# LingmaFuture/PRCV2025REID

Hardware: AMD Instinct MI355X
Metric: multimodal instances/sec (PxK, 5-modality) at 1/2/4/8 GPU; eval queries/sec (higher is better)
Workload: dtype bf16

## Files before the change

### prcv2025reid_amd/csrc/common.h

```cpp
#pragma once
#include <hip/hip_runtime.h>
#include <stdint.h>
#include <stdio.h>
#include "../../include/reid_hip.h"

typedef __attribute__((ext_vector_type(8))) short bf16x8;
typedef __attribute__((ext_vector_type(4))) short bf16x4;
typedef __attribute__((ext_vector_type(4))) float f32x4;
typedef __attribute__((ext_vector_type(16))) float f32x16;
typedef unsigned short bf16_t;

__attribute__((visibility("hidden"))) void reid_set_error(const char* fmt, ...);

enum reid_knob_id { KNOB_GEMM_TILE, KNOB_ATTN_BWD, KNOB_LORA_IMPL, KNOB_LN_IMPL, KNOB_TOPK_TILE, KNOB_TOPK_SCAN, KNOB_COUNT };
__attribute__((visibility("hidden"))) int reid_knob(int id);
__attribute__((visibility("hidden"))) int reid_num_cus();

#define REID_CHECK_ARG(cond, ...)                     \
    do {                                              \
        if (!(cond)) {                                \
            reid_set_error(__VA_ARGS__);              \
            return REID_ERR_ARG;                      \
        }                                             \
    } while (0)

static inline hipError_t reid_max_dyn_lds(const void* fn, int bytes, unsigned* done_mask) {
    int dev = 0;
    hipError_t e = hipGetDevice(&dev);
    if (e != hipSuccess) return e;
    if (dev >= 0 && dev < 32 && ((__atomic_load_n(done_mask, __ATOMIC_ACQUIRE) >> dev) & 1u)) return hipSuccess;
    e = hipFuncSetAttribute(fn, hipFuncAttributeMaxDynamicSharedMemorySize, bytes);
    if (e == hipSuccess && dev >= 0 && dev < 32) __atomic_fetch_or(done_mask, 1u << dev, __ATOMIC_RELEASE);
    return e;
}
#define REID_MAX_LDS(kernel, bytes)                                                                              \
    do {                                                                                                         \
        static unsigned lds_done_ = 0;                                                                           \
        const hipError_t le_ = reid_max_dyn_lds((const void*)(kernel), (int)(bytes), &lds_done_);                \
        if (le_ != hipSuccess) {                                                                                 \
            reid_set_error("hipFuncSetAttribute(%s, dynamic LDS %d): %s", #kernel, (int)(bytes), hipGetErrorString(le_)); \
            return REID_ERR_LAUNCH;                                                                              \
        }                                                                                                        \
    } while (0)

#define REID_CHECK_HIP(call, what)                                                     \
    do {                                                                               \
        const hipError_t he_ = (call);                                                 \
        if (he_ != hipSuccess) {                                                       \
            reid_set_error("%s: %s", what, hipGetErrorString(he_));                    \
            return REID_ERR_LAUNCH;                                                    \
        }                                                                              \
    } while (0)

#define REID_CHECK_LAUNCH(name)                                                        \
    do {                                                                               \
        hipError_t e_ = hipGetLastError();                                             \
        if (e_ != hipSuccess) {                                                        \
            reid_set_error("%s: launch failed: %s", name, hipGetErrorString(e_));     \
            return REID_ERR_LAUNCH;                                                    \
        }                                                                              \
    } while (0)

typedef _Float16 __attribute__((ext_vector_type(8))) half8_t;
#ifdef REID_FLAVOR_F16
__device__ __forceinline__ float bf16_to_f32(bf16_t v) { return (float)__builtin_bit_cast(_Float16, v); }
__device__ __forceinline__ bf16_t f32_to_bf16(float f) { return __builtin_bit_cast(bf16_t, (_Float16)f); }
__device__ __forceinline__ f32x4 mfma16(bf16x8 a, bf16x8 b, f32x4 c) {
    return __builtin_amdgcn_mfma_f32_16x16x32_f16(__builtin_bit_cast(half8_t, a), __builtin_bit_cast(half8_t, b), c, 0, 0, 0);
}
__device__ __forceinline__ f32x16 mfma32(bf16x8 a, bf16x8 b, f32x16 c) {
    return __builtin_amdgcn_mfma_f32_32x32x16_f16(__builtin_bit_cast(half8_t, a), __builtin_bit_cast(half8_t, b), c, 0, 0, 0);
}
#define REID_T16_ENTER() __builtin_amdgcn_s_setreg(1 | (23 << 6) | (0 << 11), 1)
#define REID_FLAVOR_ID 1
#define REID_T16_EPS 0.0009765625f
#else
__device__ __forceinline__ float bf16_to_f32(bf16_t v) { return __uint_as_float(((uint32_t)v) << 16); }
__device__ __forceinline__ bf16_t f32_to_bf16(float f) {
    __bf16 b = (__bf16)f;
    return __builtin_bit_cast(bf16_t, b);
}
__device__ __forceinline__ f32x4 mfma16(bf16x8 a, bf16x8 b, f32x4 c) { return __builtin_amdgcn_mfma_f32_16x16x32_bf16(a, b, c, 0, 0, 0); }
__device__ __forceinline__ f32x16 mfma32(bf16x8 a, bf16x8 b, f32x16 c) { return __builtin_amdgcn_mfma_f32_32x32x16_bf16(a, b, c, 0, 0, 0); }
#define REID_T16_ENTER() do { } while (0)
#define REID_FLAVOR_ID 0
#define REID_T16_EPS 0.00390625f
#endif

typedef float pk_f32x2 __attribute__((ext_vector_type(2)));
#ifdef REID_FLAVOR_F16
typedef _Float16 pk_t16x2 __attribute__((ext_vector_type(2)));
#else
typedef __bf16 pk_t16x2 __attribute__((ext_vector_type(2)));
#endif
__device__ __forceinline__ uint32_t pack_bf16x2(float lo, float hi) {
    const pk_t16x2 r = __builtin_convertvector(pk_f32x2{lo, hi}, pk_t16x2);
    return __builtin_bit_cast(uint32_t, r);
}

typedef _Float16 pk_h16x2 __attribute__((ext_vector_type(2)));
__device__ __forceinline__ uint32_t pack_f16x2(float lo, float hi) {
    const pk_h16x2 r = __builtin_convertvector(pk_f32x2{lo, hi}, pk_h16x2);
    return __builtin_bit_cast(uint32_t, r);
}
__device__ __forceinline__ float f16_to_f32(unsigned short v) { return (float)__builtin_bit_cast(_Float16, v); }
#define REID_F16_SATURATE() __builtin_amdgcn_s_setreg(1 | (23 << 6) | (0 << 11), 1)
__device__ __forceinline__ bool f16_clamps(float v) { const float a = fabsf(v); return a >= 65520.f && a <= 3.402823466e38f; }

__device__ __forceinline__ float wave_sum(float v) {
#pragma unroll
    for (int o = 32; o > 0; o >>= 1) v += __shfl_xor(v, o, 64);
    return v;
}
__device__ __forceinline__ float wave_max(float v) {
#pragma unroll
    for (int o = 32; o > 0; o >>= 1) v = fmaxf(v, __shfl_xor(v, o, 64));
    return v;
}

__device__ __forceinline__ void gauss_cdf_pdf(float x, float& cdf, float& pdf_unnorm) {
    const float z = fabsf(x) * 0.70710678118654752f;
    const float t = __builtin_amdgcn_rcpf(fmaf(0.3275911f, z, 1.0f));
    const float e = __builtin_amdgcn_exp2f(x * x * -0.72134752044448170f);
    const float poly = t * fmaf(t, fmaf(t, fmaf(t, fmaf(t, 1.061405429f, -1.453152027f), 1.421413741f), -0.284496736f), 0.254829592f);
    const float q = 0.5f * poly * e;
    cdf = x >= 0.f ? 1.0f - q : q;
    pdf_unnorm = e;
}
__device__ __forceinline__ float gelu_erf_f(float x) {
    float c, e;
    gauss_cdf_pdf(x, c, e);
    return x * c;
}
__device__ __forceinline__ void gelu_both_f(float x, float& g, float& dg) {
    float c, e;
    gauss_cdf_pdf(x, c, e);
    g = x * c;
    dg = fmaf(x * 0.39894228040143268f, e, c);
}
typedef float f32x2_t __attribute__((ext_vector_type(2)));
__device__ __forceinline__ void gelu_both_x2(f32x2_t x, f32x2_t& g, f32x2_t& dg) {
    const f32x2_t xs = (x * x) * -0.72134752044448170f;
    f32x2_t e; e.x = __builtin_amdgcn_exp2f(xs.x); e.y = __builtin_amdgcn_exp2f(xs.y);
    f32x2_t z; z.x = __builtin_fabsf(x.x); z.y = __builtin_fabsf(x.y);
    const f32x2_t den = z * (0.3275911f * 0.70710678118654752f) + 1.0f;
    f32x2_t t; t.x = __builtin_amdgcn_rcpf(den.x); t.y = __builtin_amdgcn_rcpf(den.y);
    f32x2_t poly = t * (0.5f * 1.061405429f) + (0.5f * -1.453152027f);
    poly = poly * t + (0.5f * 1.421413741f);
    poly = poly * t + (0.5f * -0.284496736f);
    poly = poly * t + (0.5f * 0.254829592f);
    const f32x2_t q = (poly * t) * e;
    const f32x2_t h = 0.5f - q;
    f32x2_t sh; sh.x = __builtin_copysignf(h.x, x.x); sh.y = __builtin_copysignf(h.y, x.y);
    const f32x2_t cdf = sh + 0.5f;
    g = x * cdf;
    dg = (x * 0.39894228040143268f) * e + cdf;
}
__device__ __forceinline__ float dgelu_erf_f(float x) {
    float c, e;
    gauss_cdf_pdf(x, c, e);
    return fmaf(x * 0.39894228040143268f, e, c);
}
__device__ __forceinline__ float quick_gelu_f(float x) { return x / (1.0f + __expf(-1.702f * x)); }
__device__ __forceinline__ float dquick_gelu_f(float x) {
    const float s = 1.0f / (1.0f + __expf(-1.702f * x));
    return s + x * 1.702f * s * (1.0f - s);
}
// ... 1 lines not shown
```

### prcv2025reid_amd/csrc/gemm.hip

```cpp
#include "gemm_core.h"
#include <stdlib.h>
#include <type_traits>

namespace {

struct GemmParams {
    const bf16_t* A; const bf16_t* B; const bf16_t* A2; const bf16_t* B2;
    const float* bias; const void* R; const bf16_t* aux;
    void* C; void* C2;
    const int32_t* img_mod;
    const float* row_scale;
    int M, N, K, K2;
    int lda, ldb, lda2, ldb2, ldr, ldaux, ldc, ldc2;
    int k2_group_n;
    int act, c_dtype, c2_dtype, r_dtype;
    int r_period;
    int mask_r, mask_period, rows_per_img;
    int c_group, c_group_stride, c_row_off;
    float alpha;
    int tiles_m, tiles_n;
    int group_m;
    int perm_b;
    int epi;
    int n_groups;
// ... 301 lines not shown
    if (!p.perm_b || p.R || p.row_scale) return EPI_GENERIC;
    if (p.act == REID_ACT_NONE && !p.C2 && !p.aux) return p.c_dtype == REID_F16 ? EPI_PLAIN16H : EPI_PLAIN16;
    if (p.act == REID_ACT_GELU_ERF && p.C2 && p.c2_dtype != REID_F32 && !p.aux) return EPI_GELU2;
    if (p.act == REID_ACT_DGELU_ERF && p.aux && !p.C2) return EPI_DGELU;
    if (p.act == REID_ACT_GELU_ERF_DSAVE && p.C2 && p.c2_dtype != REID_F32 && !p.aux) return EPI_GELU2D;
    if (p.act == REID_ACT_MUL_AUX && p.aux && !p.C2) return EPI_MULAUX;
    return EPI_GENERIC;
}

__host__ __device__ inline bool epilogue_wide16(const GemmParams& p) {
    return p.c_dtype != REID_F32 && ((p.N | p.ldc) & 7) == 0 && (!p.C2 || (p.ldc2 & 7) == 0) && (!p.R || (p.ldr & 7) == 0) &&
           (!p.aux || (p.ldaux & 7) == 0);
}

template <int TM, int TN>
__device__ __forceinline__ void store_tile(const GemmParams& p, f32x4 (&acc)[TN][TM], int m_base, int n_base, int lane, int m_end) {
    if (p.c_dtype == REID_F32) store_tile_m<TM, TN, 0>(p, acc, m_base, n_base, lane, m_end);
    else if (p.perm_b) store_tile_m<TM, TN, 1>(p, acc, m_base, n_base, lane, m_end);
    else store_tile_m<TM, TN, 2>(p, acc, m_base, n_base, lane, m_end);
}

template <int BM, int BN, int WM, int WN, int EPI = EPI_GENERIC>
__global__ __launch_bounds__(WM* WN * 64, 2) void mer_gemm_kernel(const GemmParams p) {
    REID_T16_ENTER();
    using C = Cfg<BM, BN, WM, WN>;
    if constexpr (EPI == EPI_PLAIN16H) REID_F16_SATURATE();
    extern __shared__ __attribute__((aligned(16))) char smem[];
    const int tid = threadIdx.x;
    const int lane = tid & 63;
    const int wave = __builtin_amdgcn_readfirstlane(tid >> 6);
    const int wm = wave / WN, wn = wave % WN;

    const int lin = xcd_linear_block(blockIdx.x, gridDim.x);
    int tm, tn;
    tile_coords(lin, p.tiles_m, p.tiles_n, tm, tn, p.group_m);
    int m0, m_end;
    const bf16_t* Bw;
    tile_rows(p, tm, BM, m0, m_end, Bw);
    const int n0 = tn * BN;
    const int g = (p.k2_group_n > 0) ? (n0 / p.k2_group_n) : 0;
    const bf16_t* A2 = p.A2 ? p.A2 + (size_t)g * p.K2 : nullptr;

    f32x4 acc[C::TN][C::TM];
    if constexpr (EPI == EPI_GENERIC) init_acc<C::TM, C::TN>(p, acc, n0 + wn * (BN / WN), lane);
    else if constexpr (EPI == EPI_RES32) init_acc_m<C::TM, C::TN, 0>(p, acc, n0 + wn * (BN / WN), lane);
    else init_acc_m<C::TM, C::TN, 1>(p, acc, n0 + wn * (BN / WN), lane);
    mainloop<BM, BN, WM, WN>(p.A, p.lda, Bw, p.ldb, A2, p.lda2, p.B2, p.ldb2, m_end, p.N, p.K, p.K2, m0, n0, smem, acc,
                             p.perm_b != 0);

    constexpr int WTM = BM / WM, WTN = BN / WN;
    if constexpr (EPI == EPI_GENERIC) store_tile<C::TM, C::TN>(p, acc, m0 + wm * WTM, n0 + wn * WTN, lane, m_end);
    else store_tile_fast<C::TM, C::TN, EPI>(p, acc, m0 + wm * WTM, n0 + wn * WTN, lane, m_end);
}

template <int EPI, int BM = 256>
__global__ __launch_bounds__(512, 2) void mer_gemm_pp_kernel(const GemmParams p) {
    REID_T16_ENTER();
    if constexpr (EPI == EPI_PLAIN16H) REID_F16_SATURATE();
    using PC = PPCfg<BM, 256>;
    constexpr int TM = PC::TM, RW = PC::RW;
    extern __shared__ __attribute__((aligned(16))) char smem[];
    const int tid = threadIdx.x;
    const int lane = tid & 63;
    const int wave = __builtin_amdgcn_readfirstlane(tid >> 6);
    const int wm = wave >> 2, wn = wave & 3;
#ifdef REID_GEMM_TRACE
#define GEMM_TRACE(slot) do { if (p.trace && threadIdx.x == 0) p.trace[(size_t)blockIdx.x * 8 + (slot)] = __builtin_amdgcn_s_memrealtime(); } while (0)
    if (p.trace && threadIdx.x == 0) p.trace[(size_t)blockIdx.x * 8 + 6] = ((unsigned long long)__builtin_amdgcn_s_getreg(20 | (0 << 6) | (31 << 11)) << 32) | __builtin_amdgcn_s_getreg(4 | (0 << 6) | (31 << 11));
#else
#define GEMM_TRACE(slot) do { } while (0)
#endif
    GEMM_TRACE(0);
    const int lin = xcd_linear_block(blockIdx.x, gridDim.x);
    int tm, tn;
    tile_coords(lin, p.tiles_m, p.tiles_n, tm, tn, p.group_m);
    int m0, m_end;
    const bf16_t* Bw;
    tile_rows(p, tm, BM, m0, m_end, Bw);
    const int n0 = tn * 256;
    const int g = (p.k2_group_n > 0) ? (n0 / p.k2_group_n) : 0;
    const bf16_t* A2 = p.A2 ? p.A2 + (size_t)g * p.K2 : nullptr;
    f32x4 acc[4][TM];
    if constexpr (EPI == EPI_GENERIC) init_acc<TM, 4>(p, acc, n0 + wn * 64, lane);
    else if constexpr (EPI == EPI_RES32) init_acc_m<TM, 4, 0>(p, acc, n0 + wn * 64, lane);
    else init_acc_m<TM, 4, 1>(p, acc, n0 + wn * 64, lane);
    constexpr bool AUX_IN_LOOP = EPI == EPI_MULAUX && BM == 256;
    const bool aux_staged = AUX_IN_LOOP && p.K2 == 0 && (p.K >> 6) >= 2;
    mainloop_pp<BM, 256, AUX_IN_LOOP>(p.A, p.lda, Bw, p.ldb, A2, p.lda2, p.B2, p.ldb2, m_end, p.N, p.K, p.K2, m0, n0, smem, acc, p.perm_b != 0,
                                      aux_staged ? (const bf16_t*)p.aux : nullptr, p.ldaux);
    GEMM_TRACE(1);
    if constexpr (EPI == EPI_MULAUX) {
        if (aux_staged) {
            asm volatile("s_waitcnt vmcnt(0)" ::: "memory");
            __syncthreads();
            store_tile_fast<TM, 4, EPI>(p, acc, m0 + wm * RW, n0 + wn * 64, lane, m_end, smem, wm * RW, wn * 8);
            GEMM_TRACE(2);
#ifdef REID_GEMM_TRACE
            asm volatile("s_waitcnt vmcnt(0)" ::: "memory");
            GEMM_TRACE(3);
#endif
            return;
        }
        __syncthreads();
#pragma unroll
        for (int q = 0; q < BM / 16; ++q) {
            const int rp = q * 8 + wave;
            const int row = 2 * rp + (lane >> 5);
            const int c = lane & 31;
            const int gm = m0 + row < m_end ? m0 + row : m_end - 1;
            const char* src = (const char*)p.aux + ((size_t)gm * p.ldaux + n0) * 2 + ((c ^ (row & 15)) << 4);
            __builtin_amdgcn_global_load_lds((gptr_t)src, (lptr_t)(smem + rp * 1024), 16, 0, 0);
        }
        asm volatile("s_waitcnt vmcnt(0)" ::: "memory");
        __syncthreads();
        store_tile_fast<TM, 4, EPI>(p, acc, m0 + wm * RW, n0 + wn * 64, lane, m_end, smem, wm * RW, wn * 8);
        GEMM_TRACE(2);
#ifdef REID_GEMM_TRACE
        asm volatile("s_waitcnt vmcnt(0)" ::: "memory");
        GEMM_TRACE(3);
#endif
        return;
    }
    if constexpr (EPI == EPI_GENERIC) store_tile<TM, 4>(p, acc, m0 + wm * RW, n0 + wn * 64, lane, m_end);
    else store_tile_fast<TM, 4, EPI>(p, acc, m0 + wm * RW, n0 + wn * 64, lane, m_end);
    GEMM_TRACE(2);
#ifdef REID_GEMM_TRACE
    asm volatile("s_waitcnt vmcnt(0)" ::: "memory");
    GEMM_TRACE(3);
#endif
}
#ifdef REID_GEMM_TRACE
static unsigned long long* g_gemm_trace = nullptr;
extern "C" void reid_debug_gemm_trace(void* buf) { g_gemm_trace = (unsigned long long*)buf; }
#endif

template <int EPI, int BM = 256>
__global__ __launch_bounds__(512, 2) void mer_gemm_pps_kernel(const GemmParams p) {
    REID_T16_ENTER();
    if constexpr (EPI == EPI_PLAIN16H) REID_F16_SATURATE();
    using PC = PPCfg<BM, 256>;
    constexpr int TM = PC::TM, RW = PC::RW;
    extern __shared__ __attribute__((aligned(16))) char smem[];
    const int lane = threadIdx.x & 63;
    const int wave = __builtin_amdgcn_readfirstlane(threadIdx.x >> 6);
    const int wm = wave >> 2, wn = wave & 3;
    const int n_tiles = p.tiles_m * p.tiles_n;
    auto tile_of = [&](int v, int& m0, int& m_end, int& n0, const bf16_t*& Bw) {
        const int lin = xcd_linear_block(v, n_tiles);
        int tm, tn;
        tile_coords(lin, p.tiles_m, p.tiles_n, tm, tn, p.group_m);
        tile_rows(p, tm, BM, m0, m_end, Bw);
        n0 = tn * 256;
    };
    auto init = [&](f32x4 (&acc)[4][TM], int n0) {
        if constexpr (EPI == EPI_RES32) init_acc_m<TM, 4, 0>(p, acc, n0 + wn * 64, lane);
        else init_acc_m<TM, 4, 1>(p, acc, n0 + wn * 64, lane);
    };
    auto epi = [&](f32x4 (&acc)[4][TM], int m0, int m_end, int n0) {
        store_tile_fast<TM, 4, EPI>(p, acc, m0 + wm * RW, n0 + wn * 64, lane, m_end);
    };
#ifdef REID_GEMM_TRACE
    auto trace = [&](int v, int slot) {
        if (!p.trace) return;
        if (threadIdx.x == 0) {
            p.trace[(size_t)v * 8 + slot] = __builtin_amdgcn_s_memrealtime();
#ifndef REID_GEMM_TRACE_CLOCK
            if (slot == 0) p.trace[(size_t)v * 8 + 7] = ((unsigned long long)__builtin_amdgcn_s_getreg(20 | (0 << 6) | (31 << 11)) << 32) | __builtin_amdgcn_s_getreg(4 | (0 << 6) | (31 << 11));
#endif
        }
#ifdef REID_GEMM_TRACE_CLOCK
        if (threadIdx.x == 0 && slot == 1) p.trace[(size_t)v * 8 + 6] = __builtin_amdgcn_s_memtime();
        if (threadIdx.x == 0 && slot == 2) p.trace[(size_t)v * 8 + 7] = __builtin_amdgcn_s_memtime();
#else
        if (threadIdx.x == 256 && slot == 5) p.trace[(size_t)v * 8 + 6] = __builtin_amdgcn_s_memrealtime();
#endif
    };
#else
    auto trace = [&](int, int) {};
#endif
    stream_pp<BM, 256>(p.A, p.lda, p.ldb, p.N, p.K, n_tiles, smem, p.perm_b != 0, tile_of, init, epi, trace);
}

template <int EPI, int BM>
int launch_pps_e(GemmParams& p, hipStream_t s) {
    using C = PPCfg<BM, 256>;
    constexpr int LDS = C::LDS_BYTES;
    REID_MAX_LDS((mer_gemm_pps_kernel<EPI, BM>), LDS);
    const int tiles = p.tiles_m * p.tiles_n;
    int grid = reid_num_cus() & ~7;
    if (grid > tiles) grid = tiles;
#ifdef REID_GEMM_TRACE
    p.trace = g_gemm_trace;
#endif
    hipLaunchKernelGGL((mer_gemm_pps_kernel<EPI, BM>), dim3(grid), dim3(C::NT), LDS, s, p);
    REID_CHECK_LAUNCH("reid_mer_gemm");
    return REID_OK;
}


template <int EPI, int BM>
int launch_pp_e(GemmParams& p, hipStream_t s) {
    using C = PPCfg<BM, 256>;
    REID_MAX_LDS((mer_gemm_pp_kernel<EPI, BM>), C::LDS_BYTES);
    hipLaunchKernelGGL((mer_gemm_pp_kernel<EPI, BM>), dim3(p.tiles_m * p.tiles_n), dim3(C::NT), C::LDS_BYTES, s, p);
    REID_CHECK_LAUNCH("reid_mer_gemm");
    return REID_OK;
}
static int pick_pp_bm(const GemmParams& p, int tile_knob) {
    if (tile_knob == 12) return 256;
    if (tile_knob == 14) return 224;
    const long cus = reid_num_cus();
    const long tn = p.N / 256;
    GemmParams q = p;
    const long t256 = (long)row_tiles(q, 256, false) * tn, t224 = (long)row_tiles(q, 224, false) * tn;
    return (t224 + cus - 1) / cus <= (t256 + cus - 1) / cus ? 224 : 256;
}
int launch_pp(GemmParams& p, hipStream_t s, int tile_knob) {
    p.epi = pick_epilogue(p, 256);
    const int bm = p.epi == EPI_GENERIC ? 256 : pick_pp_bm(p, tile_knob);
    p.tiles_m = row_tiles(p, bm, true);
    p.tiles_n = (p.N + 255) / 256;
#ifdef REID_GEMM_TRACE
    p.trace = g_gemm_trace;
#endif
    if (p.K2 == 0 && p.K >= 192 && (reid_num_cus() & ~7) >= 8) {
        switch (p.epi) {
            case EPI_PLAIN16: return bm == 224 ? launch_pps_e<EPI_PLAIN16, 224>(p, s) : launch_pps_e<EPI_PLAIN16, 256>(p, s);
#ifndef REID_FLAVOR_F16
            case EPI_PLAIN16H: return bm == 224 ? launch_pps_e<EPI_PLAIN16H, 224>(p, s) : launch_pps_e<EPI_PLAIN16H, 256>(p, s);
#endif
            case EPI_RES32: return bm == 224 ? launch_pps_e<EPI_RES32, 224>(p, s) : launch_pps_e<EPI_RES32, 256>(p, s);
            default: break;
        }
    }
#define REID_PP_CASE(E) case E: return bm == 224 ? launch_pp_e<E, 224>(p, s) : launch_pp_e<E, 256>(p, s);
    switch (p.epi) {
        REID_PP_CASE(EPI_PLAIN16)
#ifndef REID_FLAVOR_F16
        REID_PP_CASE(EPI_PLAIN16H)
#endif
        REID_PP_CASE(EPI_RES32)
        REID_PP_CASE(EPI_GELU2)
        REID_PP_CASE(EPI_DGELU)
        REID_PP_CASE(EPI_GELU2D)
        REID_PP_CASE(EPI_MULAUX)
        default: return launch_pp_e<EPI_GENERIC, 256>(p, s);
    }
#undef REID_PP_CASE
}

template <int BM, int BN, int WM, int WN, int EPI>
int launch_e(GemmParams& p, hipStream_t s) {
    using C = Cfg<BM, BN, WM, WN>;
    REID_MAX_LDS((mer_gemm_kernel<BM, BN, WM, WN, EPI>), C::LDS_BYTES);
    hipLaunchKernelGGL((mer_gemm_kernel<BM, BN, WM, WN, EPI>), dim3(p.tiles_m * p.tiles_n), dim3(C::NT), C::LDS_BYTES, s, p);
    REID_CHECK_LAUNCH("reid_mer_gemm");
    return REID_OK;
}
int launch_main(GemmParams& p, hipStream_t s) {
    p.tiles_m = row_tiles(p, 128, true);
    p.tiles_n = (p.N + 127) / 128;
    p.epi = pick_epilogue(p, 128);
    switch (p.epi) {
        case EPI_PLAIN16: return launch_e<128, 128, 2, 2, EPI_PLAIN16>(p, s);
#ifndef REID_FLAVOR_F16
        case EPI_PLAIN16H: return launch_e<128, 128, 2, 2, EPI_PLAIN16H>(p, s);
#endif
        case EPI_RES32: return launch_e<128, 128, 2, 2, EPI_RES32>(p, s);
        case EPI_GELU2: return launch_e<128, 128, 2, 2, EPI_GELU2>(p, s);
        case EPI_DGELU: return launch_e<128, 128, 2, 2, EPI_DGELU>(p, s);
        case EPI_GELU2D: return launch_e<128, 128, 2, 2, EPI_GELU2D>(p, s);
        case EPI_MULAUX: return launch_e<128, 128, 2, 2, EPI_MULAUX>(p, s);
        default: return launch_e<128, 128, 2, 2, EPI_GENERIC>(p, s);
    }
}

template <int BM, int BN, int WM, int WN>
int launch(GemmParams& p, hipStream_t s) {
    using C = Cfg<BM, BN, WM, WN>;
    p.tiles_m = row_tiles(p, BM, true);
    p.tiles_n = (p.N + BN - 1) / BN;
    REID_MAX_LDS((mer_gemm_kernel<BM, BN, WM, WN>), C::LDS_BYTES);
    const int grid = p.tiles_m * p.tiles_n;
    hipLaunchKernelGGL((mer_gemm_kernel<BM, BN, WM, WN>), dim3(grid), dim3(C::NT), C::LDS_BYTES, s, p);
    REID_CHECK_LAUNCH("reid_mer_gemm");
    return REID_OK;
}

}

extern "C" int reid_mer_gemm(const reid_gemm_args* a, void* stream) {
    REID_CHECK_ARG(a != nullptr, "reid_mer_gemm: null args");
    REID_CHECK_ARG(a->A && a->B && a->C, "reid_mer_gemm: A, B, C must be non-null");
    REID_CHECK_ARG(a->M > 0 && a->N > 0 && a->K > 0, "reid_mer_gemm: empty problem M=%d N=%d K=%d", a->M, a->N, a->K);
    REID_CHECK_ARG(a->K % 64 == 0, "reid_mer_gemm: K=%d must be a multiple of 64", a->K);
    REID_CHECK_ARG(a->N % 4 == 0, "reid_mer_gemm: N=%d must be a multiple of 4", a->N);
    REID_CHECK_ARG(a->lda >= a->K && a->ldb >= a->K && a->lda % 8 == 0 && a->ldb % 8 == 0,
                   "reid_mer_gemm: lda/ldb must be >= K and multiples of 8 (16-byte rows)");
    REID_CHECK_ARG(a->ldc >= a->N && a->ldc % 4 == 0, "reid_mer_gemm: ldc=%d", a->ldc);
    REID_CHECK_ARG((int64_t)a->M * a->lda * 2 < (1ll << 32) && (int64_t)a->N * a->ldb * 2 < (1ll << 32),
                   "reid_mer_gemm: operands beyond 4 GiB need 64-bit lane offsets (M*lda=%lld)", (long long)a->M * a->lda);
    if (a->A2) {
        REID_CHECK_ARG(a->B2 && a->K2 > 0 && a->K2 % 32 == 0, "reid_mer_gemm: K2=%d must be a positive multiple of 32",
                       a->K2);
        REID_CHECK_ARG(a->lda2 % 8 == 0 && a->ldb2 % 8 == 0 && a->ldb2 >= a->K2, "reid_mer_gemm: lda2/ldb2");
        const int groups = a->k2_group_n > 0 ? (a->N + a->k2_group_n - 1) / a->k2_group_n : 1;
        REID_CHECK_ARG(a->lda2 >= groups * a->K2, "reid_mer_gemm: lda2=%d < groups*K2=%d", a->lda2, groups * a->K2);
        REID_CHECK_ARG(a->k2_group_n == 0 || a->k2_group_n % 128 == 0, "reid_mer_gemm: k2_group_n must be a multiple of 128");
    }
    REID_CHECK_ARG(a->act >= 0 && a->act <= REID_ACT_GELU_ERF_DSAVE, "reid_mer_gemm: act=%d", a->act);
    REID_CHECK_ARG(a->act < REID_ACT_DGELU_ERF || a->act > REID_ACT_MUL_AUX || (a->aux && a->ldaux >= a->N), "reid_mer_gemm: D* / MUL_AUX activation needs aux");
    REID_CHECK_ARG(a->act != REID_ACT_GELU_ERF_DSAVE || a->C2, "reid_mer_gemm: GELU_ERF_DSAVE needs C2");
    REID_CHECK_ARG(!a->R || a->ldr >= a->N, "reid_mer_gemm: ldr");
    REID_CHECK_ARG(!a->C2 || a->ldc2 >= a->N, "reid_mer_gemm: ldc2");
    REID_CHECK_ARG(a->mask_r == 0 || (a->img_mod && a->rows_per_img > 0 && a->mask_period > 0),
                   "reid_mer_gemm: modality mask needs img_mod, rows_per_img, mask_period");
    REID_CHECK_ARG(a->c_group == 0 || a->c_group_stride >= a->c_group, "reid_mer_gemm: c_group_stride");
    REID_CHECK_ARG(!a->row_scale || a->rows_per_img > 0, "reid_mer_gemm: row_scale needs rows_per_img");
    REID_CHECK_ARG(a->n_row_groups >= 0 && a->n_row_groups <= REID_GEMM_MAX_GROUPS, "reid_mer_gemm: n_row_groups=%d (max %d)", a->n_row_groups, REID_GEMM_MAX_GROUPS);
    if (a->n_row_groups > 0) {
        int prev = 0;
        for (int g = 0; g < a->n_row_groups; ++g) {
            REID_CHECK_ARG(a->row_group_end[g] > prev, "reid_mer_gemm: row_group_end must be strictly increasing (empty groups are left out by the caller)");
            REID_CHECK_ARG(a->row_group_b[g] >= 0, "reid_mer_gemm: row_group_b[%d] < 0", g);
            REID_CHECK_ARG((int64_t)(a->row_group_b[g] + 1) * a->b_group_stride * 2 < (1ll << 40), "reid_mer_gemm: weight stack too large");
            prev = a->row_group_end[g];
        }
        REID_CHECK_ARG(prev == a->M, "reid_mer_gemm: the row groups must cover exactly M=%d rows (last end %d)", a->M, prev);
        REID_CHECK_ARG(a->b_group_stride >= (int64_t)a->N * a->ldb, "reid_mer_gemm: b_group_stride smaller than one [N, ldb] matrix");
        REID_CHECK_ARG(a->c_group == 0 && a->r_period == 0, "reid_mer_gemm: row groups do not combine with c_group / r_period");
    }
    GemmParams p;
    p.trace = nullptr;
    p.A = (const bf16_t*)a->A; p.B = (const bf16_t*)a->B; p.A2 = (const bf16_t*)a->A2; p.B2 = (const bf16_t*)a->B2;
    p.bias = a->bias; p.R = a->R; p.aux = (const bf16_t*)a->aux; p.C = a->C; p.C2 = a->C2; p.img_mod = a->img_mod; p.row_scale = a->row_scale;
    p.M = a->M; p.N = a->N; p.K = a->K; p.K2 = a->A2 ? a->K2 : 0;
    p.n_groups = a->n_row_groups;
    p.b_group_stride = a->b_group_stride;
    for (int g = 0; g < REID_GEMM_MAX_GROUPS; ++g) {
        p.grp_row0[g] = p.grp_row_end[g] = p.grp_tile0[g] = p.grp_b[g] = 0;
        if (g < a->n_row_groups) {
            p.grp_row0[g] = g == 0 ? 0 : a->row_group_end[g - 1];
            p.grp_row_end[g] = a->row_group_end[g];
            p.grp_b[g] = a->row_group_b[g];
        }
    }
    p.lda = a->lda; p.ldb = a->ldb; p.lda2 = a->lda2; p.ldb2 = a->ldb2; p.ldr = a->ldr; p.ldaux = a->ldaux;
    p.ldc = a->ldc; p.ldc2 = a->ldc2; p.k2_group_n = a->k2_group_n;
    p.act = a->act; p.c_dtype = a->c_dtype; p.c2_dtype = a->c2_dtype; p.r_dtype = a->r_dtype;
    p.r_period = a->r_period; p.mask_r = a->mask_r; p.mask_period = a->mask_period; p.rows_per_img = a->rows_per_img;
    p.c_group = a->c_group; p.c_group_stride = a->c_group_stride; p.c_row_off = a->c_row_off;
    p.alpha = a->alpha == 0.f ? 1.f : a->alpha;
    if (p.c_dtype == REID_F16 && REID_FLAVOR_ID == 1) p.c_dtype = REID_BF16;
    REID_CHECK_ARG(!(a->C2 && a->c2_dtype == REID_F16 && REID_FLAVOR_ID == 0) && !(a->R && a->r_dtype == REID_F16 && REID_FLAVOR_ID == 0),
                   "reid_mer_gemm: REID_F16 is supported for C only");
    p.group_m = 8;
    p.perm_b = epilogue_wide16(p) ? 1 : 0;
    hipStream_t s = (hipStream_t)stream;
    if (p.c_dtype == REID_F16) {
        REID_CHECK_ARG(a->N > 96 && a->N % 128 == 0 && reid_knob(KNOB_GEMM_TILE) <= 0 &&
                       pick_epilogue(p, 128) == EPI_PLAIN16H,
                       "reid_mer_gemm: a REID_F16 output needs the plain 16-bit epilogue (N a multiple of 128, no activation / residual / second output / mask / row remap)");
    }
    if (a->N <= 32) return a->M >= 65536 ? launch<256, 32, 4, 1>(p, s) : launch<64, 32, 4, 1>(p, s);
    if (a->N <= 64) return a->M >= 65536 ? launch<256, 64, 4, 1>(p, s) : launch<64, 64, 4, 1>(p, s);
    if (a->N <= 96) return launch<128, 32, 4, 1>(p, s);
    const int tile = reid_knob(KNOB_GEMM_TILE) > 0 ? reid_knob(KNOB_GEMM_TILE) : 0;
    if (tile == 3) return launch_main(p, s);
    {
        const bool pp_ok = (p.k2_group_n == 0 || p.k2_group_n % 256 == 0) && p.N % 256 == 0;
        const long tiles256 = (long)row_tiles(p, 256, false) * (p.N / 256);
        const bool pp_shape = tiles256 >= reid_num_cus();
        if (pp_ok && (tile == 12 || tile == 14 || (tile == 0 && pp_shape && pick_epilogue(p, 256) != EPI_GENERIC)))
            return launch_pp(p, s, tile);
    }
    return launch_main(p, s);
}
```

### prcv2025reid_amd/csrc/gemm_core.h

```cpp
#pragma once
#include "common.h"
#include <type_traits>

namespace gemmcore {

__device__ __forceinline__ int swz(int row, int c) { return c ^ ((row >> 1) & 7); }

typedef const __attribute__((address_space(1))) void* gptr_t;
typedef __attribute__((address_space(3))) void* lptr_t;

template <int BM, int BN, int WM, int WN>
struct Cfg {
    static constexpr int NW = WM * WN;
    static constexpr int NT = NW * 64;
    static constexpr int TM = BM / WM / 16;
    static constexpr int TN = BN / WN / 16;
    static constexpr int A_BYTES = BM * 128;
    static constexpr int B_BYTES = BN * 128;
    static constexpr int BUF_BYTES = A_BYTES + B_BYTES;
    static constexpr int LDS_BYTES = 2 * BUF_BYTES;
    static constexpr int A_INSTR = BM / 8 / NW;
    static constexpr int B_INSTR = BN / 8 / NW;
    static_assert(BM % (8 * NW) == 0 && BN % (8 * NW) == 0, "tile rows must split over waves");
};
// ... 171 lines not shown
        for (int j = 0; j < 2; ++j) {
            const int r = (j * 8 + wave) * 8 + rl;
            const int rb = 128 * h + r;
            int gb = n0 + (perm_b ? perm32(rb) : rb);
            gb = gb < N - 1 ? gb : N - 1;
            offB[h][j] = (uint32_t)gb * (uint32_t)ldb * 2u + (uint32_t)swz(r, cl) * 16u;
        }
    auto stage_a = [&](int t, int buf) {
        char* dst = smem + buf * C::BUF_BYTES + wm * C::HALF_BYTES;
        const char* src = (const char*)A + (size_t)t * 128;
#pragma unroll
        for (int j = 0; j < 3; ++j)
            __builtin_amdgcn_global_load_lds((gptr_t)(src + offA[j]), (lptr_t)(dst + (j * 4 + wn) * 8 * 128), 16, 0, 0);
        if (C::A_INSTR == 16 || a_last)
            __builtin_amdgcn_global_load_lds((gptr_t)(src + offA[3]), (lptr_t)(dst + (12 + wn) * 8 * 128), 16, 0, 0);
    };
    auto stage_b = [&](int t, int buf) {
        const char* src = (const char*)B + (size_t)t * 128;
#pragma unroll
        for (int h = 0; h < 2; ++h)
#pragma unroll
            for (int j = 0; j < 2; ++j)
                __builtin_amdgcn_global_load_lds((gptr_t)(src + offB[h][j]),
                                                 (lptr_t)(smem + buf * C::BUF_BYTES + (2 + h) * C::HALF_BYTES + (j * 8 + wave) * 8 * 128), 16, 0, 0);
    };
    auto stage_a2 = [&](int t, int buf) {
        char* dst = smem + buf * C::BUF_BYTES + wm * C::HALF_BYTES;
        const int k2 = (t - nk) << 5;
#pragma unroll
        for (int j = 0; j < 4; ++j) {
            if (j == 3 && C::A_INSTR != 16 && !a_last) break;
            const int r = (j * 4 + wn) * 8 + rl;
            int ga = m0 + C::RW * wm + r;
            ga = ga < M - 1 ? ga : M - 1;
            const bf16_t* g = A2 + (size_t)ga * lda2 + k2 + (swz(r, cl) & 3) * 8;
            __builtin_amdgcn_global_load_lds((gptr_t)g, (lptr_t)(dst + (j * 4 + wn) * 8 * 128), 16, 0, 0);
        }
    };
    auto stage_b2 = [&](int t, int buf) {
        const int k2 = (t - nk) << 5;
#pragma unroll
        for (int h = 0; h < 2; ++h)
#pragma unroll
            for (int j = 0; j < 2; ++j) {
                const int r = (j * 8 + wave) * 8 + rl;
                const int rb = 128 * h + r;
                int gb = n0 + (perm_b ? perm32(rb) : rb);
                gb = gb < N - 1 ? gb : N - 1;
                const bf16_t* g = B2 + (size_t)gb * ldb2 + k2 + (swz(r, cl) & 3) * 8;
                __builtin_amdgcn_global_load_lds((gptr_t)g, (lptr_t)(smem + buf * C::BUF_BYTES + (2 + h) * C::HALF_BYTES + (j * 8 + wave) * 8 * 128), 16, 0, 0);
            }
    };
    auto stage_aux_piece = [&](int rp, char* dst) {
        const int row = 2 * rp + (lane >> 5), c = lane & 31;
        const int gm = m0 + row < M ? m0 + row : M - 1;
        const char* src = (const char*)aux + ((size_t)gm * ldaux + n0) * 2 + ((c ^ (row & 15)) << 4);
        __builtin_amdgcn_global_load_lds((gptr_t)src, (lptr_t)dst, 16, 0, 0);
    };
    auto stage_aux_b = [&](int buf) {
#pragma unroll
        for (int h = 0; h < 2; ++h)
#pragma unroll
            for (int j = 0; j < 2; ++j)
                stage_aux_piece(buf * 64 + (2 + h) * 16 + j * 8 + wave, smem + buf * C::BUF_BYTES + (2 + h) * C::HALF_BYTES + (j * 8 + wave) * 1024);
    };
    auto stage_aux_a = [&](int buf) {
#pragma unroll
        for (int j = 0; j < 4; ++j)
            stage_aux_piece(buf * 64 + wm * 16 + j * 4 + wn, smem + buf * C::BUF_BYTES + wm * C::HALF_BYTES + (j * 4 + wn) * 1024);
    };
    const bool aux_on = AUXPRE && aux != nullptr && nt >= 2;
    auto stage_a_any = [&](int t, int buf) { if (t < nk) stage_a(t, buf); else stage_a2(t, buf); };
    auto stage_b_any = [&](int t, int buf) { if (t < nk) stage_b(t, buf); else stage_b2(t, buf); };

    const int frow = lane & 15, fq = lane >> 4;
    int foff[2];
#pragma unroll
    for (int ks = 0; ks < 2; ++ks) foff[ks] = frow * 128 + ((swz(frow, ks * 4 + fq)) << 4);
    const int a_base = wm * C::HALF_BYTES;
    const int b_base = (2 + (wn >> 1)) * C::HALF_BYTES + (wn & 1) * 64 * 128;
    bf16x8 af[4][2], bfr[2][2][2];
    auto read_a = [&](int buf, int a, auto nks_c) {
        constexpr int NKS = decltype(nks_c)::value;
        const char* base = smem + buf * C::BUF_BYTES + a_base + a * 64 * 128;
#pragma unroll
        for (int i = 0; i < 4; ++i) {
            if (a == 1 && i >= C::TM1) break;
#pragma unroll
            for (int ks = 0; ks < NKS; ++ks) af[i][ks] = *(const bf16x8*)(base + i * 16 * 128 + foff[ks]);
        }
    };
    auto read_b = [&](int buf, auto nks_c) {
        constexpr int NKS = decltype(nks_c)::value;
        const char* base = smem + buf * C::BUF_BYTES + b_base;
#pragma unroll
        for (int b = 0; b < 2; ++b)
#pragma unroll
            for (int j = 0; j < 2; ++j)
#pragma unroll
                for (int ks = 0; ks < NKS; ++ks) bfr[b][j][ks] = *(const bf16x8*)(base + (b * 32 + j * 16) * 128 + foff[ks]);
    };
    auto half = [&](auto a_c, auto nks_c) {
        constexpr int NKS = decltype(nks_c)::value, a = decltype(a_c)::value;
        __builtin_amdgcn_s_setprio(1);
#pragma unroll
        for (int ks = 0; ks < NKS; ++ks)
#pragma unroll
            for (int b = 0; b < 2; ++b)
#pragma unroll
                for (int j = 0; j < 2; ++j)
#pragma unroll
                    for (int i = 0; i < (a == 0 ? C::TM0 : C::TM1); ++i)
                        acc[2 * b + j][4 * a + i] = mfma16(bfr[b][j][ks], af[i][ks], acc[2 * b + j][4 * a + i]);
        __builtin_amdgcn_s_setprio(0);
    };
    auto bar = [&]() {
        __builtin_amdgcn_sched_barrier(0);
        __builtin_amdgcn_s_barrier();
        __builtin_amdgcn_sched_barrier(0);
    };
    using I0 = std::integral_constant<int, 0>; using I1 = std::integral_constant<int, 1>; using I2 = std::integral_constant<int, 2>;
    auto ktile = [&](int T, int cur, auto nks_c, auto fast_c) {
        constexpr bool FAST = decltype(fast_c)::value != 0;
        read_a(cur, 0, nks_c); read_b(cur, nks_c);
        pp_wait_lgkm0(); bar();
        half(I0{}, nks_c); bar();
        read_a(cur, 1, nks_c);
        if constexpr (FAST) { stage_b(T + 2, cur); pp_wait_vm4(); }
        else if (T + 2 < nt) { stage_b_any(T + 2, cur); pp_wait_vm4(); }
        else if (AUXPRE && aux_on) { stage_aux_b(cur); pp_wait_vm4(); }
        else { pp_wait_vm0(); }
        pp_wait_lgkm0(); bar();
        if constexpr (FAST) stage_a(T + 2, cur); else if (T + 2 < nt) stage_a_any(T + 2, cur); else if (AUXPRE && aux_on) stage_aux_a(cur);
        half(I1{}, nks_c); bar();
    };

    stage_b_any(0, 0); stage_a_any(0, 0);
    if (nt > 1) {
        stage_b_any(1, 1); stage_a_any(1, 1);
        if (C::A_INSTR == 16 || a_last) asm volatile("s_waitcnt vmcnt(8)" ::: "memory");
        else asm volatile("s_waitcnt vmcnt(7)" ::: "memory");
    } else { pp_wait_vm0(); }
    bar();
    if (wm == 1) bar();
    int cur = 0;
    int T = 0;
    for (; T + 2 < nk; ++T) { ktile(T, cur, I2{}, I1{}); cur ^= 1; }
    for (; T < nk; ++T) { ktile(T, cur, I2{}, I0{}); cur ^= 1; }
    for (; T < nt; ++T) { ktile(T, cur, I1{}, I0{}); cur ^= 1; }
    if (wm == 0) bar();
}


template <int BM, int BN, typename TileOf, typename InitAcc, typename Epilogue, typename Trace>
__device__ __forceinline__ void stream_pp(const bf16_t* __restrict__ A, int lda, int ldb, int N, int K, int n_tiles, char* smem,
                                          bool perm_b, TileOf tile_of, InitAcc init_acc, Epilogue epilogue, Trace trace) {
    using C = PPCfg<BM, BN>;
    const int tid = threadIdx.x;
    const int lane = tid & 63;
    const int wave = __builtin_amdgcn_readfirstlane(tid >> 6);
    const int wm = wave >> 2, wn = wave & 3;
    const int nk = K >> 6;
    const int rl = lane >> 3, cl = lane & 7;
    const bool a_last = 12 + wn < C::A_INSTR;

    int m0 = 0, m_end = 0, n0 = 0;
    const bf16_t* Bt = nullptr;
    const bf16_t* Bw = nullptr;
    uint32_t offA[4], offB[2][2];
    auto set_offsets = [&]() {
        Bw = Bt;
        const int ln = __builtin_amdgcn_mbcnt_hi(~0u, __builtin_amdgcn_mbcnt_lo(~0u, 0u));
        const int rl = ln >> 3, cl = ln & 7;
#pragma unroll
        for (int j = 0; j < 4; ++j) {
            const int r = (j * 4 + wn) * 8 + rl;
            int ga = m0 + C::RW * wm + r;
            ga = ga < m_end - 1 ? ga : m_end - 1;
            offA[j] = (uint32_t)ga * (uint32_t)lda * 2u + (uint32_t)swz(r, cl) * 16u;
        }
#pragma unroll
        for (int h = 0; h < 2; ++h)
#pragma unroll
            for (int j = 0; j < 2; ++j) {
                const int r = (j * 8 + wave) * 8 + rl;
                const int rb = 128 * h + r;
                int gb = n0 + (perm_b ? perm32(rb) : rb);
                gb = gb < N - 1 ? gb : N - 1;
                offB[h][j] = (uint32_t)gb * (uint32_t)ldb * 2u + (uint32_t)swz(r, cl) * 16u;
            }
    };
    auto stage_a = [&](int t, int buf) {
        char* dst = smem + buf * C::BUF_BYTES + wm * C::HALF_BYTES;
        const char* src = (const char*)A + (size_t)t * 128;
#pragma unroll
        for (int j = 0; j < 3; ++j)
            __builtin_amdgcn_global_load_lds((gptr_t)(src + offA[j]), (lptr_t)(dst + (j * 4 + wn) * 8 * 128), 16, 0, 0);
        if (C::A_INSTR == 16 || a_last)
            __builtin_amdgcn_global_load_lds((gptr_t)(src + offA[3]), (lptr_t)(dst + (12 + wn) * 8 * 128), 16, 0, 0);
    };
    auto stage_b = [&](int t, int buf) {
        const char* src = (const char*)Bw + (size_t)t * 128;
#pragma unroll
        for (int h = 0; h < 2; ++h)
#pragma unroll
            for (int j = 0; j < 2; ++j)
                __builtin_amdgcn_global_load_lds((gptr_t)(src + offB[h][j]),
                                                 (lptr_t)(smem + buf * C::BUF_BYTES + (2 + h) * C::HALF_BYTES + (j * 8 + wave) * 8 * 128), 16, 0, 0);
    };
    const int frow = lane & 15, fq = lane >> 4;
    int foff[2];
#pragma unroll
    for (int ks = 0; ks < 2; ++ks) foff[ks] = frow * 128 + ((swz(frow, ks * 4 + fq)) << 4);
    const int a_base = wm * C::HALF_BYTES;
    const int b_base = (2 + (wn >> 1)) * C::HALF_BYTES + (wn & 1) * 64 * 128;
    f32x4 acc[4][C::TM];
    bf16x8 af[4][2], bfr[2][2][2];
    auto read_a = [&](int buf, int a) {
        const char* base = smem + buf * C::BUF_BYTES + a_base + a * 64 * 128;
#pragma unroll
        for (int i = 0; i < 4; ++i) {
            if (a == 1 && i >= C::TM1) break;
#pragma unroll
            for (int ks = 0; ks < 2; ++ks) af[i][ks] = *(const bf16x8*)(base + i * 16 * 128 + foff[ks]);
        }
    };
    auto read_b = [&](int buf) {
        const char* base = smem + buf * C::BUF_BYTES + b_base;
#pragma unroll
        for (int b = 0; b < 2; ++b)
#pragma unroll
            for (int j = 0; j < 2; ++j)
#pragma unroll
                for (int ks = 0; ks < 2; ++ks) bfr[b][j][ks] = *(const bf16x8*)(base + (b * 32 + j * 16) * 128 + foff[ks]);
    };
    auto half = [&](auto a_c) {
        constexpr int a = decltype(a_c)::value;
        __builtin_amdgcn_s_setprio(1);
#pragma unroll
        for (int ks = 0; ks < 2; ++ks)
#pragma unroll
            for (int b = 0; b < 2; ++b)
#pragma unroll
                for (int j = 0; j < 2; ++j)
#pragma unroll
                    for (int i = 0; i < (a == 0 ? C::TM0 : C::TM1); ++i)
                        acc[2 * b + j][4 * a + i] = mfma16(bfr[b][j][ks], af[i][ks], acc[2 * b + j][4 * a + i]);
        __builtin_amdgcn_s_setprio(0);
    };
    auto bar = [&]() {
        __builtin_amdgcn_sched_barrier(0);
        __builtin_amdgcn_s_barrier();
        __builtin_amdgcn_sched_barrier(0);
    };
    using I0 = std::integral_constant<int, 0>; using I1 = std::integral_constant<int, 1>;
    auto ktile = [&](int cur, int st) {
        read_a(cur, 0); read_b(cur);
        pp_wait_lgkm0(); bar();
        half(I0{}); bar();
        read_a(cur, 1);
        if (st >= 0) { stage_b(st, cur); pp_wait_vm4(); } else { pp_wait_vm0(); }
        pp_wait_lgkm0(); bar();
        if (st >= 0) stage_a(st, cur);
        half(I1{}); bar();
    };
    auto ktile_fast = [&](int cur, int st) {
        read_a(cur, 0); read_b(cur);
        pp_wait_lgkm0(); bar();
        half(I0{}); bar();
        read_a(cur, 1);
        stage_b(st, cur); pp_wait_vm4();
        pp_wait_lgkm0(); bar();
        stage_a(st, cur);
        half(I1{}); bar();
    };

    int v = blockIdx.x;
    tile_of(v, m0, m_end, n0, Bt);
    set_offsets();
    stage_b(0, 0); stage_a(0, 0);
    stage_b(1, 1); stage_a(1, 1);
    if (C::A_INSTR == 16 || a_last) asm volatile("s_waitcnt vmcnt(8)" ::: "memory");
    else asm volatile("s_waitcnt vmcnt(7)" ::: "memory");
    bar();
    int cur = 0;
    for (;;) {
        if (wm == 1) bar();
        const int cm0 = m0, cm_end = m_end, cn0 = n0;
        trace(v, 0);
        init_acc(acc, cn0);
        trace(v, 1);
        constexpr bool EARLY = BM < 256;
        const int vn = v + (int)gridDim.x;
        const bool has_next = vn < n_tiles;
        if (EARLY && has_next) tile_of(vn, m0, m_end, n0, Bt);
        for (int T = 0; T + 2 < nk; ++T) { ktile_fast(cur, T + 2); cur ^= 1; }
        trace(v, 2);
        if (!EARLY && has_next) tile_of(vn, m0, m_end, n0, Bt);
        if (has_next) set_offsets();
        trace(v, 3);
        ktile(cur, has_next ? 0 : -1); cur ^= 1;
        ktile(cur, has_next ? 1 : -1); cur ^= 1;
        if (wm == 0) bar();
        trace(v, 4);
        epilogue(acc, cm0, cm_end, cn0);
        trace(v, 5);
        if (!has_next) break;
        v = vn;
    }
}


}
```

### prcv2025reid_amd/csrc/rowops.hip

```cpp
#include "common.h"
#include <stdarg.h>
#include <string.h>
#include <stdlib.h>

static thread_local char g_err[512] = "";
void reid_set_error(const char* fmt, ...) {
    va_list ap;
    va_start(ap, fmt);
    vsnprintf(g_err, sizeof(g_err), fmt, ap);
    va_end(ap);
}
extern "C" const char* reid_last_error(void) { return g_err; }
extern "C" int reid_version(void) { return REID_ABI_VERSION; }

static const char* const g_knob_names[] = {"GEMM_TILE", "ATTN_BWD", "LORA_IMPL", "LN_IMPL", "TOPK_TILE", "TOPK_SCAN"};
static_assert(sizeof(g_knob_names) / sizeof(g_knob_names[0]) == KNOB_COUNT, "one name per reid_knob_id");
static int g_knobs[KNOB_COUNT];
static int* knob_table() {
    static const bool init = [] {
        for (int i = 0; i < KNOB_COUNT; ++i) {
            char name[64];
            snprintf(name, sizeof(name), "REID_%s", g_knob_names[i]);
            const char* e = getenv(name);
            g_knobs[i] = e ? atoi(e) : -1;
        }
        return true;
    }();
    (void)init;
    return g_knobs;
}
int reid_knob(int id) { return knob_table()[id]; }
extern "C" int reid_set_knob(const char* name, int value) {
    int* t = knob_table();
    for (int i = 0; i < KNOB_COUNT; ++i)
        if (strcmp(name, g_knob_names[i]) == 0) {
            t[i] = value; return REID_OK;
        }
    reid_set_error("reid_set_knob: unknown knob %s", name);
    return REID_ERR_ARG;
}
int reid_num_cus() {
    static const int n = [] {
        int dev = 0;
        hipDeviceProp_t prop;
        if (hipGetDevice(&dev) != hipSuccess || hipGetDeviceProperties(&prop, dev) != hipSuccess) return 256;
        return prop.multiProcessorCount > 0 ? prop.multiProcessorCount : 256;
    }();
    return n;
}
extern "C" int reid_flavor(void) { return REID_FLAVOR_ID; }
extern "C" int reid_check_device(int dev) {
    hipDeviceProp_t prop;
    if (hipGetDeviceProperties(&prop, dev) != hipSuccess) {
        reid_set_error("reid_check_device: hipGetDeviceProperties(%d) failed", dev);
        return REID_ERR_DEVICE;
    }
    if (strncmp(prop.gcnArchName, "gfx950", 6) != 0) {
        reid_set_error("reid_check_device: device %d is %s, this library is built for gfx950 only", dev, prop.gcnArchName);
        return REID_ERR_DEVICE;
    }
    return REID_OK;
}

namespace {

constexpr int MAXV = 4;

__global__ __launch_bounds__(256) void ln_fwd_kernel(const float* __restrict__ x, int ldx, const int32_t* __restrict__ row_index,
                                                     const float* __restrict__ gamma, const float* __restrict__ beta,
                                                     bf16_t* __restrict__ yb, float* __restrict__ yf, int ldy,
                                                     float* __restrict__ mean, float* __restrict__ rstd, int rows,
                                                     int cols, float eps) {
    REID_T16_ENTER();
    const int lane = threadIdx.x & 63;
    const int row = blockIdx.x * 4 + (threadIdx.x >> 6);
    if (row >= rows) return;
    const size_t src = row_index ? (size_t)row_index[row] : (size_t)row;
    const float* xr = x + src * ldx;
    const int nv = cols >> 2;
    f32x4 v[MAXV];
    float s = 0.f;
#pragma unroll
    for (int i = 0; i < MAXV; ++i) {
        const int c = lane + i * 64;
        v[i] = c < nv ? *(const f32x4*)(xr + c * 4) : f32x4{0.f, 0.f, 0.f, 0.f};
        s += v[i][0] + v[i][1] + v[i][2] + v[i][3];
    }
    const float mu = wave_sum(s) / cols;
    float q = 0.f;
#pragma unroll
    for (int i = 0; i < MAXV; ++i) {
        const int c = lane + i * 64;
        if (c < nv) {
#pragma unroll
            for (int e = 0; e < 4; ++e) { const float d = v[i][e] - mu; q += d * d; }
        }
    }
    const float rs = rsqrtf(wave_sum(q) / cols + eps);
    if (lane == 0) {
        if (mean) mean[row] = mu;
        if (rstd) rstd[row] = rs;
    }
#pragma unroll
    for (int i = 0; i < MAXV; ++i) {
        const int c = lane + i * 64;
        if (c < nv) {
            const f32x4 g = *(const f32x4*)(gamma + c * 4);
            const f32x4 b = *(const f32x4*)(beta + c * 4);
            f32x4 o;
#pragma unroll
            for (int e = 0; e < 4; ++e) o[e] = (v[i][e] - mu) * rs * g[e] + b[e];
            if (yf) *(f32x4*)(yf + (size_t)row * ldy + c * 4) = o;
            if (yb) *(uint2*)(yb + (size_t)row * ldy + c * 4) = uint2{pack_bf16x2(o[0], o[1]), pack_bf16x2(o[2], o[3])};
        }
    }
}

template <bool Y_HALF>
__global__ __launch_bounds__(256) void add_ln_fwd_kernel(const float* __restrict__ x, int ldx, const bf16_t* __restrict__ y, int ldy,
                                                         const float* __restrict__ row_scale, int rows_per_img,
                                                         float* __restrict__ xo, int ldxo, const float* __restrict__ gamma,
                                                         const float* __restrict__ beta, bf16_t* __restrict__ hb, int ldh,
                                                         float* __restrict__ mean, float* __restrict__ rstd, int rows, int cols, float eps) {
    REID_T16_ENTER();
    const int lane = threadIdx.x & 63;
    const int row = blockIdx.x * 4 + (threadIdx.x >> 6);
    if (row >= rows) return;
    const float* xr = x + (size_t)row * ldx;
    const bf16_t* yr = y + (size_t)row * ldy;
    const float sc = row_scale ? row_scale[row / rows_per_img] : 1.f;
    const int nv = cols >> 2;
    f32x4 v[MAXV];
    float s = 0.f;
#pragma unroll
    for (int i = 0; i < MAXV; ++i) {
        const int c = lane + i * 64;
        if (c < nv) {
            const f32x4 a = *(const f32x4*)(xr + c * 4);
            const bf16x4 b = *(const bf16x4*)(yr + c * 4);
#pragma unroll
            for (int e = 0; e < 4; ++e) v[i][e] = fmaf(sc, Y_HALF ? f16_to_f32((unsigned short)b[e]) : bf16_to_f32((bf16_t)b[e]), a[e]);
            *(f32x4*)(xo + (size_t)row * ldxo + c * 4) = v[i];
        } else {
            v[i] = f32x4{0.f, 0.f, 0.f, 0.f};
        }
        s += v[i][0] + v[i][1] + v[i][2] + v[i][3];
    }
    const float mu = wave_sum(s) / cols;
    float q = 0.f;
#pragma unroll
    for (int i = 0; i < MAXV; ++i) {
        const int c = lane + i * 64;
        if (c < nv) {
#pragma unroll
            for (int e = 0; e < 4; ++e) { const float d = v[i][e] - mu; q += d * d; }
        }
    }
    const float rs = rsqrtf(wave_sum(q) / cols + eps);
    if (lane == 0) {
        if (mean) mean[row] = mu;
        if (rstd) rstd[row] = rs;
    }
#pragma unroll
    for (int i = 0; i < MAXV; ++i) {
        const int c = lane + i * 64;
        if (c < nv) {
            const f32x4 g = *(const f32x4*)(gamma + c * 4);
            const f32x4 b = *(const f32x4*)(beta + c * 4);
// ... 462 lines not shown
```

Baseline: 2136.

## Route GELU GEMM epilogue through persistent ping-pong kernel with LDS-staged bias

Adds a knob-gated path that sends bias+GELU GEMMs to the persistent streaming ping-pong kernel instead of the generic kernel. Bias for the next tile is prefetched into a per-wave LDS slot with async global-to-LDS loads and used to initialise accumulators. Vector-memory wait placement is changed: a full drain at the start, no wait on the first fast k-tile, and a drain before the epilogue when a next tile exists. This costs extra LDS per block and some wait conservatism, which could reduce overlap.

```diff
diff --git a/prcv2025reid_amd/csrc/common.h b/prcv2025reid_amd/csrc/common.h
--- a/prcv2025reid_amd/csrc/common.h
+++ b/prcv2025reid_amd/csrc/common.h
@@ -12,7 +12,7 @@
 
 __attribute__((visibility("hidden"))) void reid_set_error(const char* fmt, ...);
 
-enum reid_knob_id { KNOB_GEMM_TILE, KNOB_ATTN_BWD, KNOB_LORA_IMPL, KNOB_LN_IMPL, KNOB_TOPK_TILE, KNOB_TOPK_SCAN, KNOB_COUNT };
+enum reid_knob_id { KNOB_GEMM_TILE, KNOB_ATTN_BWD, KNOB_LORA_IMPL, KNOB_LN_IMPL, KNOB_TOPK_TILE, KNOB_TOPK_SCAN, KNOB_GEMM_GELU_PPS, KNOB_COUNT };
 __attribute__((visibility("hidden"))) int reid_knob(int id);
 __attribute__((visibility("hidden"))) int reid_num_cus();
 
diff --git a/prcv2025reid_amd/csrc/gemm.hip b/prcv2025reid_amd/csrc/gemm.hip
--- a/prcv2025reid_amd/csrc/gemm.hip
+++ b/prcv2025reid_amd/csrc/gemm.hip
@@ -477,9 +477,14 @@
         tile_rows(p, tm, BM, m0, m_end, Bw);
         n0 = tn * 256;
     };
-    auto init = [&](f32x4 (&acc)[4][TM], int n0) {
-        if constexpr (EPI == EPI_RES32) init_acc_m<TM, 4, 0>(p, acc, n0 + wn * 64, lane);
-        else init_acc_m<TM, 4, 1>(p, acc, n0 + wn * 64, lane);
+    auto init = [&](f32x4 (&acc)[4][TM], const char* bias_slot) {
+        const int fq = lane >> 4;
+#pragma unroll
+        for (int j = 0; j < 4; ++j) {
+            const f32x4 b = bias_slot ? *(const f32x4*)(bias_slot + 4 * acc_col<EPI == EPI_RES32 ? 0 : 1>(j, 0, fq)) : f32x4{0.f, 0.f, 0.f, 0.f};
+#pragma unroll
+            for (int i = 0; i < TM; ++i) acc[j][i] = b;
+        }
     };
     auto epi = [&](f32x4 (&acc)[4][TM], int m0, int m_end, int n0) {
         store_tile_fast<TM, 4, EPI>(p, acc, m0 + wm * RW, n0 + wn * 64, lane, m_end);
@@ -503,13 +508,13 @@
 #else
     auto trace = [&](int, int) {};
 #endif
-    stream_pp<BM, 256>(p.A, p.lda, p.ldb, p.N, p.K, n_tiles, smem, p.perm_b != 0, tile_of, init, epi, trace);
+    stream_pp<BM, 256>(p.A, p.lda, p.ldb, p.N, p.K, n_tiles, smem, p.perm_b != 0, p.bias, tile_of, init, epi, trace);
 }
 
 template <int EPI, int BM>
 int launch_pps_e(GemmParams& p, hipStream_t s) {
     using C = PPCfg<BM, 256>;
-    constexpr int LDS = C::LDS_BYTES;
+    constexpr int LDS = C::LDS_BYTES + PPS_BIAS_BYTES;
     REID_MAX_LDS((mer_gemm_pps_kernel<EPI, BM>), LDS);
     const int tiles = p.tiles_m * p.tiles_n;
     int grid = reid_num_cus() & ~7;
@@ -548,6 +553,7 @@
 #ifdef REID_GEMM_TRACE
     p.trace = g_gemm_trace;
 #endif
+    const bool gelu_pps = reid_knob(KNOB_GEMM_GELU_PPS) != 0;
     if (p.K2 == 0 && p.K >= 192 && (reid_num_cus() & ~7) >= 8) {
         switch (p.epi) {
             case EPI_PLAIN16: return bm == 224 ? launch_pps_e<EPI_PLAIN16, 224>(p, s) : launch_pps_e<EPI_PLAIN16, 256>(p, s);
@@ -555,6 +561,9 @@
             case EPI_PLAIN16H: return bm == 224 ? launch_pps_e<EPI_PLAIN16H, 224>(p, s) : launch_pps_e<EPI_PLAIN16H, 256>(p, s);
 #endif
             case EPI_RES32: return bm == 224 ? launch_pps_e<EPI_RES32, 224>(p, s) : launch_pps_e<EPI_RES32, 256>(p, s);
+            case EPI_GELU2D:
+                if (gelu_pps) return bm == 224 ? launch_pps_e<EPI_GELU2D, 224>(p, s) : launch_pps_e<EPI_GELU2D, 256>(p, s);
+                break;
             default: break;
         }
     }
diff --git a/prcv2025reid_amd/csrc/gemm_core.h b/prcv2025reid_amd/csrc/gemm_core.h
--- a/prcv2025reid_amd/csrc/gemm_core.h
+++ b/prcv2025reid_amd/csrc/gemm_core.h
@@ -347,9 +347,11 @@
 }
 
 
+constexpr int PPS_BIAS_BYTES = 8 * 1024;
 template <int BM, int BN, typename TileOf, typename InitAcc, typename Epilogue, typename Trace>
 __device__ __forceinline__ void stream_pp(const bf16_t* __restrict__ A, int lda, int ldb, int N, int K, int n_tiles, char* smem,
-                                          bool perm_b, TileOf tile_of, InitAcc init_acc, Epilogue epilogue, Trace trace) {
+                                          bool perm_b, const float* __restrict__ bias, TileOf tile_of, InitAcc init_acc, Epilogue epilogue,
+                                          Trace trace) {
     using C = PPCfg<BM, BN>;
     const int tid = threadIdx.x;
     const int lane = tid & 63;
@@ -403,6 +405,12 @@
                 __builtin_amdgcn_global_load_lds((gptr_t)(src + offB[h][j]),
                                                  (lptr_t)(smem + buf * C::BUF_BYTES + (2 + h) * C::HALF_BYTES + (j * 8 + wave) * 8 * 128), 16, 0, 0);
     };
+    char* const bias_slot = smem + C::LDS_BYTES + wave * 1024;
+    auto stage_bias = [&]() {
+        if (!bias) return;
+        const int ln = __builtin_amdgcn_mbcnt_hi(~0u, __builtin_amdgcn_mbcnt_lo(~0u, 0u));
+        __builtin_amdgcn_global_load_lds((gptr_t)(bias + n0 + wn * 64 + (ln & 15) * 4), (lptr_t)bias_slot, 16, 0, 0);
+    };
     const int frow = lane & 15, fq = lane >> 4;
     int foff[2];
 #pragma unroll
@@ -454,17 +462,19 @@
         pp_wait_lgkm0(); bar();
         half(I0{}); bar();
         read_a(cur, 1);
+        if (st == 1) stage_bias();
         if (st >= 0) { stage_b(st, cur); pp_wait_vm4(); } else { pp_wait_vm0(); }
         pp_wait_lgkm0(); bar();
         if (st >= 0) stage_a(st, cur);
         half(I1{}); bar();
     };
-    auto ktile_fast = [&](int cur, int st) {
+    auto ktile_fast = [&](int cur, int st, auto wait_c) {
         read_a(cur, 0); read_b(cur);
         pp_wait_lgkm0(); bar();
         half(I0{}); bar();
         read_a(cur, 1);
-        stage_b(st, cur); pp_wait_vm4();
+        stage_b(st, cur);
+        if constexpr (decltype(wait_c)::value != 0) pp_wait_vm4();
         pp_wait_lgkm0(); bar();
         stage_a(st, cur);
         half(I1{}); bar();
@@ -473,23 +483,24 @@
     int v = blockIdx.x;
     tile_of(v, m0, m_end, n0, Bt);
     set_offsets();
+    stage_bias();
     stage_b(0, 0); stage_a(0, 0);
     stage_b(1, 1); stage_a(1, 1);
-    if (C::A_INSTR == 16 || a_last) asm volatile("s_waitcnt vmcnt(8)" ::: "memory");
-    else asm volatile("s_waitcnt vmcnt(7)" ::: "memory");
+    pp_wait_vm0();
     bar();
     int cur = 0;
     for (;;) {
         if (wm == 1) bar();
         const int cm0 = m0, cm_end = m_end, cn0 = n0;
         trace(v, 0);
-        init_acc(acc, cn0);
+        init_acc(acc, bias ? bias_slot : nullptr);
         trace(v, 1);
         constexpr bool EARLY = BM < 256;
         const int vn = v + (int)gridDim.x;
         const bool has_next = vn < n_tiles;
         if (EARLY && has_next) tile_of(vn, m0, m_end, n0, Bt);
-        for (int T = 0; T + 2 < nk; ++T) { ktile_fast(cur, T + 2); cur ^= 1; }
+        ktile_fast(cur, 2, I0{}); cur ^= 1;
+        for (int T = 1; T + 2 < nk; ++T) { ktile_fast(cur, T + 2, I1{}); cur ^= 1; }
         trace(v, 2);
         if (!EARLY && has_next) tile_of(vn, m0, m_end, n0, Bt);
         if (has_next) set_offsets();
@@ -497,6 +508,7 @@
         ktile(cur, has_next ? 0 : -1); cur ^= 1;
         ktile(cur, has_next ? 1 : -1); cur ^= 1;
         if (wm == 0) bar();
+        if (has_next) pp_wait_vm0();
         trace(v, 4);
         epilogue(acc, cm0, cm_end, cn0);
         trace(v, 5);
diff --git a/prcv2025reid_amd/csrc/rowops.hip b/prcv2025reid_amd/csrc/rowops.hip
--- a/prcv2025reid_amd/csrc/rowops.hip
+++ b/prcv2025reid_amd/csrc/rowops.hip
@@ -13,7 +13,7 @@
 extern "C" const char* reid_last_error(void) { return g_err; }
 extern "C" int reid_version(void) { return REID_ABI_VERSION; }
 
-static const char* const g_knob_names[] = {"GEMM_TILE", "ATTN_BWD", "LORA_IMPL", "LN_IMPL", "TOPK_TILE", "TOPK_SCAN"};
+static const char* const g_knob_names[] = {"GEMM_TILE", "ATTN_BWD", "LORA_IMPL", "LN_IMPL", "TOPK_TILE", "TOPK_SCAN", "GEMM_GELU_PPS"};
 static_assert(sizeof(g_knob_names) / sizeof(g_knob_names[0]) == KNOB_COUNT, "one name per reid_knob_id");
 static int g_knobs[KNOB_COUNT];
 static int* knob_table() {
```

Result: no change. 2152 (median of 6 runs) (+0.8%).
